# Etienne-bdt/Simple-VAE-RS

Hardware: NVIDIA B200
Metric: train patches/sec (64x64 SR CondVAE, device-timed) (higher is better)
Workload: dtype bf16

## Files before the change

### simple-vae-rs_b200/svrs_native/csrc/conv_simt.cu

```cuda
#include "common.cuh"
#include <stdlib.h>
#include "taps.cuh"
#include "tc_ptx.cuh"

namespace svrs {

struct ConvArgs {
    const void* in;
    void* out;
    const void* w;
    const float* bias;
    int act;
    double* bn_sums;
    TapGeom g;
};

constexpr int BK = 16;

}
#include "conv_narrow.cuh"
namespace svrs {
extern int g_tc_enabled_narrow;

template <typename T, int BM, int BN>
// ... 235 lines not shown
        if (dtype == SVRS_F32 && out_dtype == SVRS_F32) launch_pixel<float, float>(a, grid, st);
        else if (dtype == SVRS_BF16 && out_dtype == SVRS_BF16) launch_pixel<__nv_bfloat16, __nv_bfloat16>(a, grid, st);
        else if (dtype == SVRS_BF16 && out_dtype == SVRS_F32) launch_pixel<__nv_bfloat16, float>(a, grid, st);
        else { set_error("conv: unsupported (dtype, out_dtype) = (%d, %d)", dtype, out_dtype); return SVRS_E_UNSUPPORTED; }
        return check_launch("conv_pixel_kernel");
    }
    if (out_dtype != dtype || a.bn_sums) {
        set_error("conv: fp32 output / fused BatchNorm statistics are not available on the generic SIMT kernel (K=%d Nc=%d)", g.K, g.Nc);
        return SVRS_E_UNSUPPORTED;
    }
    if (g.Nc <= 16) {
        dim3 grid((unsigned)((M + 255) / 256), (g.Nc + 15) / 16, g.nprob);
        if (dtype == SVRS_F32) SVRS_LAUNCH((conv_taps_kernel<float, 256, 16>), grid, 256, 0, st, a);
        else SVRS_LAUNCH((conv_taps_kernel<__nv_bfloat16, 256, 16>), grid, 256, 0, st, a);
    } else {
        dim3 grid((unsigned)((M + 63) / 64), (g.Nc + 63) / 64, g.nprob);
        if (dtype == SVRS_F32) SVRS_LAUNCH((conv_taps_kernel<float, 64, 64>), grid, 256, 0, st, a);
        else SVRS_LAUNCH((conv_taps_kernel<__nv_bfloat16, 64, 64>), grid, 256, 0, st, a);
    }
    return check_launch("conv_taps_kernel");
}

struct WgradArgs {
    const void* gmat;
    const void* x;
    float* dw;
    int KK;
    int ksplit;
    TapGeom g;
};

}
#include "wgrad_narrow.cuh"
#include "wgrad16.cuh"
namespace svrs {

template <typename T>
__global__ void __launch_bounds__(256) wgrad_taps_kernel(const __grid_constant__ WgradArgs a) {
    pdl_entry();
    constexpr int BA = 64, BB = 64, BP = 16;
    __shared__ float Gs[BP][BA];
    __shared__ float Xs[BP][BB];
    const TapGeom& g = a.g;
    const Prob& pb = g.prob[0];
    const T* __restrict__ G = reinterpret_cast<const T*>(a.gmat) + pb.out_off;
    const T* __restrict__ X = reinterpret_cast<const T*>(a.x);
    const int Ca = g.Nc, Cb = g.K;
    const int b_tiles = (Cb + BB - 1) / BB;
    const int a0 = (blockIdx.x / b_tiles) * BA;
    const int b0 = (blockIdx.x % b_tiles) * BB;
    const int t = blockIdx.y;
    const Tap tp = pb.taps[t];
    const long long M = (long long)g.N * g.OH * g.OW;
    long long chunk = (M + a.ksplit - 1) / a.ksplit;
    chunk = (chunk + BP - 1) / BP * BP;
    const long long mbeg = (long long)blockIdx.z * chunk;
    const long long mend = mbeg + chunk < M ? mbeg + chunk : M;
    const int tid = threadIdx.x;
    const int tx = tid % 16, ty = tid / 16;
    const bool vecG = (Ca % 4 == 0), vecX = (Cb % 4 == 0);
    const int lp = tid / 16;
    const int lq = (tid % 16) * 4;

    float acc[4][4];
#pragma unroll
    for (int i = 0; i < 4; ++i)
#pragma unroll
// ... 511 lines not shown
    ConvArgs a;
    a.in = x; a.out = y; a.w = w_kn; a.bias = bias; a.act = act; a.bn_sums = bn_sums;
    geom_convT4s2(a.g, N, H, W, Cin, Cout);
    return launch_conv(a, dtype, (cudaStream_t)stream);
}

extern "C" int svrs_convT2d_fprop(const void* x, const void* w_kn, const void* w_nk, const float* bias, void* y, int dtype,
                                  int N, int H, int W, int Cin, int Cout, int act, void* stream) {
    return svrs_convT2d_fprop_ex(x, w_kn, w_nk, bias, y, dtype, nullptr, N, H, W, Cin, Cout, act, stream);
}

extern "C" int svrs_convT2d_dgrad(const void* dy, const void* w_kn, const void* w_nk, void* dx, int dtype,
                                  int N, int H, int W, int Cin, int Cout, void* stream) {
    SVRS_CHECK_ARG(dy && w_kn && dx && dtype_ok(dtype), "convT2d_dgrad: null pointer or bad dtype");
    if (N > 0 && use_tc(w_nk, dtype, Cout, Cin, W, H))
        return launch_conv_tc(2, dy, w_nk, nullptr, dx, N, 2 * H, 2 * W, Cout, Cin, SVRS_ACT_NONE, ConvExtra(), (cudaStream_t)stream);
    ConvArgs a;
    a.in = dy; a.out = dx; a.w = w_kn; a.bias = nullptr; a.act = SVRS_ACT_NONE; a.bn_sums = nullptr;
    geom_conv4s2(a.g, N, 2 * H, 2 * W, Cout, Cin);
    return launch_conv(a, dtype, (cudaStream_t)stream);
}

extern "C" int svrs_conv2d_wgrad(const void* x, const void* dy, float* dw, float* dw_packed, float* db, int dtype,
                                 int N, int H, int W, int Cin, int Cout, int ksize, int ksplit, void* stream) {
    SVRS_CHECK_ARG(x && dy && dtype_ok(dtype), "conv2d_wgrad: null pointer or bad dtype");
    SVRS_CHECK_ARG(ksize == 3 || (ksize == 4 && H % 2 == 0 && W % 2 == 0), "conv2d_wgrad: bad ksize");
    int rc = 0;
    if (dw) {
        WgradArgs a;
        a.gmat = dy; a.x = x; a.dw = dw; a.KK = ksize * ksize;
        if (ksize == 3) geom_conv3(a.g, N, H, W, Cin, Cout, false);
        else geom_conv4s2(a.g, N, H, W, Cin, Cout);
        const bool fold_db = db != nullptr && Cout % 8 == 0;
        if (g_tc_enabled_narrow && ksplit <= 0 && wgrad16_takes(dtype, N, H, W, Cin, Cout, ksize)) {
            rc = launch_wgrad16(x, dy, dw, db, N, H, W, Cin, (cudaStream_t)stream);
            db = nullptr;
        } else if (g_tc_enabled && N > 0 && dtype == SVRS_BF16 && wgrad_halo_supported(a.g, a.KK)) {
            rc = launch_wgrad3_halo(a.g, dy, x, dw_packed ? dw_packed : dw, dw_packed != nullptr, fold_db ? db : nullptr, (cudaStream_t)stream);
            if (fold_db) db = nullptr;
        } else if (g_tc_enabled && N > 0 && wgrad_tc_supported(dtype, Cout, Cin, a.g.OW, a.g.OH)) {
            rc = launch_wgrad_tc(a.g, dy, x, dw_packed ? dw_packed : dw, dw_packed != nullptr, a.KK, fold_db ? db : nullptr, (cudaStream_t)stream);
            if (fold_db) db = nullptr;
        } else if (g_tc_enabled_narrow && N > 0 && ksplit <= 0 && wgrad_narrow_mma_takes(a.g, dtype)) {
            rc = launch_wgrad_narrow_mma(a, db, (cudaStream_t)stream);
            db = nullptr;
        } else
            rc = launch_wgrad(a, dtype, ksplit, (cudaStream_t)stream);
        if (rc) return rc;
    }
    if (db) {
        int s = ksize == 3 ? 1 : 2;
        rc = launch_colsum(dy, dtype, (long long)N * (H / s) * (W / s), Cout, db, (cudaStream_t)stream);
    }
    return rc;
}

extern "C" int svrs_convT2d_wgrad(const void* x, const void* dy, float* dw, float* dw_packed, float* db, int dtype,
                                  int N, int H, int W, int Cin, int Cout, int ksplit, void* stream) {
    SVRS_CHECK_ARG(x && dy && dtype_ok(dtype), "convT2d_wgrad: null pointer or bad dtype");
    int rc = 0;
    if (dw) {
        WgradArgs a;
        a.gmat = x; a.x = dy; a.dw = dw; a.KK = 16;
        geom_conv4s2(a.g, N, 2 * H, 2 * W, Cout, Cin);
        if (g_tc_enabled && N > 0 && wgrad_tc_supported(dtype, Cin, Cout, a.g.OW, a.g.OH))
            rc = launch_wgrad_tc(a.g, x, dy, dw_packed ? dw_packed : dw, dw_packed != nullptr, 16, nullptr, (cudaStream_t)stream);
        else
            rc = launch_wgrad(a, dtype, ksplit, (cudaStream_t)stream);
        if (rc) return rc;
    }
    if (db) rc = launch_colsum(dy, dtype, (long long)N * 4 * H * W, Cout, db, (cudaStream_t)stream);
    return rc;
}

extern "C" int svrs_conv2d_wgrad_layout(int dtype, int N, int H, int W, int Cin, int Cout, int ksize) {
    if (!(ksize == 3 || (ksize == 4 && H % 2 == 0 && W % 2 == 0)) || N <= 0) return 0;
    if (g_tc_enabled_narrow && wgrad16_takes(dtype, N, H, W, Cin, Cout, ksize)) return 0;
    TapGeom g;
    if (ksize == 3) geom_conv3(g, N, H, W, Cin, Cout, false);
    else geom_conv4s2(g, N, H, W, Cin, Cout);
    if (g_tc_enabled && dtype == SVRS_BF16 && wgrad_halo_supported(g, ksize * ksize)) return 1;
    if (g_tc_enabled && wgrad_tc_supported(dtype, Cout, Cin, g.OW, g.OH)) return 1;
    return 0;
}
extern "C" int svrs_convT2d_wgrad_layout(int dtype, int N, int H, int W, int Cin, int Cout) {
    if (N <= 0) return 0;
    TapGeom g;
    geom_conv4s2(g, N, 2 * H, 2 * W, Cout, Cin);
    return (g_tc_enabled && wgrad_tc_supported(dtype, Cin, Cout, g.OW, g.OH)) ? 1 : 0;
}

extern "C" int svrs_debug_tap_geometry(int form, int N, int H, int W, int Cr, int Cw, int64_t* out, int cap) {
    SVRS_CHECK_ARG(out && form >= 0 && form <= 3, "debug_tap_geometry: bad args");
    TapGeom g;
    if (form == 0) geom_conv3(g, N, H, W, Cr, Cw, false);
    else if (form == 1) geom_conv3(g, N, H, W, Cr, Cw, true);
    else if (form == 2) geom_conv4s2(g, N, H, W, Cr, Cw);
    else geom_convT4s2(g, N, H, W, Cr, Cw);
    int n = 0;
    auto put = [&](long long v) { if (n < cap) out[n] = v; ++n; };
    put(g.N); put(g.OH); put(g.OW); put(g.IH); put(g.IW); put(g.K); put(g.Nc); put(g.nprob);
    put(g.o_sn); put(g.o_sy); put(g.o_sx); put(g.i_sn); put(g.i_sy); put(g.i_sx);
    for (int p = 0; p < g.nprob; ++p) {
        put(g.prob[p].out_off); put(g.prob[p].ntaps);
        for (int t = 0; t < g.prob[p].ntaps; ++t) {
            put(g.prob[p].taps[t].in_off); put(g.prob[p].taps[t].w_off); put(g.prob[p].taps[t].dy); put(g.prob[p].taps[t].dx);
        }
    }
    SVRS_CHECK_ARG(n <= cap, "debug_tap_geometry: buffer too small (%d needed)", n);
    return n;
// ... 2 lines not shown
```

### simple-vae-rs_b200/svrs_native/csrc/conv_tc.cu

```cuda
#include "common.cuh"
#include <stdlib.h>
#include "taps.cuh"
#include <cuda.h>
#include <string.h>
#include "tc_ptx.cuh"

namespace svrs {

constexpr int TC_STAGES = 4;
constexpr int TC_A_BYTES = 128 * 128;
constexpr int TC_B_BYTES = 256 * 128;
constexpr int TC_STAGE_BYTES = TC_A_BYTES + TC_B_BYTES;
constexpr int TC_SMEM_BYTES = TC_STAGES * TC_STAGE_BYTES + 1024  + 256 ;
constexpr int TC_THREADS = 64 + 32 * TC_EPI_WARPS;

struct TcTap {
    int map;
    int dy, dx;
    int wtap;
};
struct TcProb {
    int ntaps;
    int pad_;
    long long out_off;
// ... 162 lines not shown
        if (EXTRA && p.bn_sums) epi_bn_flush(s_bn, p.bn_sums, p.Nc, threadIdx.x - 64, 32 * TC_EPI_WARPS);
    }

    tc_fence_before();
    __syncthreads();
    if (warp == 1) {
        tc_fence_after();
        asm volatile("tcgen05.dealloc.cta_group::1.sync.aligned.b32 %0, 512;" ::"r"(tmem_base) : "memory");
    }
}

typedef CUresult (*PFN_encodeTiled)(CUtensorMap*, CUtensorMapDataType, cuuint32_t, void*, const cuuint64_t*, const cuuint64_t*,
                                    const cuuint32_t*, const cuuint32_t*, CUtensorMapInterleave, CUtensorMapSwizzle,
                                    CUtensorMapL2promotion, CUtensorMapFloatOOBfill);

static PFN_encodeTiled get_encode() {
    static PFN_encodeTiled fn = nullptr;
    if (!fn) {
        void* ptr = nullptr;
        cudaDriverEntryPointQueryResult qres;
        if (cudaGetDriverEntryPoint("cuTensorMapEncodeTiled", &ptr, cudaEnableDefault, &qres) == cudaSuccess && qres == cudaDriverEntryPointSuccess)
            fn = (PFN_encodeTiled)ptr;
    }
    return fn;
}

static CUtensorMapSwizzle swizzle_for(int cw) {
    return cw == 64 ? CU_TENSOR_MAP_SWIZZLE_128B : (cw == 32 ? CU_TENSOR_MAP_SWIZZLE_64B : CU_TENSOR_MAP_SWIZZLE_32B);
}

int chunk_width(int C) { return C % 64 == 0 ? 64 : (C % 32 == 0 ? 32 : (C % 16 == 0 ? 16 : 0)); }

int make_act_map(CUtensorMap* m, const void* base, int C, int W, int H, int N, long long sx, long long sy, long long sn,
                 int BW, int BH, int BNI, int cw) {
    PFN_encodeTiled enc = get_encode();
    if (!enc) { set_error("cuTensorMapEncodeTiled unavailable"); return SVRS_E_CUDA; }
    cuuint64_t dims[4] = {(cuuint64_t)C, (cuuint64_t)W, (cuuint64_t)H, (cuuint64_t)N};
    cuuint64_t strides[3] = {(cuuint64_t)sx * 2, (cuuint64_t)sy * 2, (cuuint64_t)sn * 2};
    cuuint32_t box[4] = {(cuuint32_t)cw, (cuuint32_t)BW, (cuuint32_t)BH, (cuuint32_t)BNI};
    cuuint32_t es[4] = {1, 1, 1, 1};
    CUresult r = enc(m, CU_TENSOR_MAP_DATA_TYPE_BFLOAT16, 4, const_cast<void*>(base), dims, strides, box, es,
                     CU_TENSOR_MAP_INTERLEAVE_NONE, swizzle_for(cw), CU_TENSOR_MAP_L2_PROMOTION_L2_128B,
                     CU_TENSOR_MAP_FLOAT_OOB_FILL_NONE);
    if (r != CUDA_SUCCESS) { set_error("cuTensorMapEncodeTiled(activation) failed: %d (C=%d W=%d H=%d N=%d cw=%d)", (int)r, C, W, H, N, cw); return SVRS_E_CUDA; }
    return 0;
}

int make_f32_2d_map(CUtensorMap* m, const void* base, long long inner, long long rows, int box_inner, int box_rows) {
    PFN_encodeTiled enc = get_encode();
    if (!enc) { set_error("cuTensorMapEncodeTiled unavailable"); return SVRS_E_CUDA; }
    cuuint64_t dims[2] = {(cuuint64_t)inner, (cuuint64_t)rows};
    cuuint64_t strides[1] = {(cuuint64_t)inner * 4};
    cuuint32_t box[2] = {(cuuint32_t)box_inner, (cuuint32_t)box_rows};
    cuuint32_t es[2] = {1, 1};
    CUtensorMapSwizzle sw = box_inner * 4 == 128 ? CU_TENSOR_MAP_SWIZZLE_128B : CU_TENSOR_MAP_SWIZZLE_64B;
    CUresult r = enc(m, CU_TENSOR_MAP_DATA_TYPE_FLOAT32, 2, const_cast<void*>(base), dims, strides, box, es,
                     CU_TENSOR_MAP_INTERLEAVE_NONE, sw, CU_TENSOR_MAP_L2_PROMOTION_NONE, CU_TENSOR_MAP_FLOAT_OOB_FILL_NONE);
    if (r != CUDA_SUCCESS) { set_error("cuTensorMapEncodeTiled(f32 2d) failed: %d (inner=%lld rows=%lld box %dx%d)", (int)r, inner, rows, box_inner, box_rows); return SVRS_E_CUDA; }
    return 0;
}

static int make_w_map(CUtensorMap* m, const void* base, int K, int Nc, int taps, int n_tile, int cw) {
    PFN_encodeTiled enc = get_encode();
    if (!enc) { set_error("cuTensorMapEncodeTiled unavailable"); return SVRS_E_CUDA; }
    cuuint64_t dims[3] = {(cuuint64_t)K, (cuuint64_t)Nc, (cuuint64_t)taps};
    cuuint64_t strides[2] = {(cuuint64_t)K * 2, (cuuint64_t)K * Nc * 2};
    cuuint32_t box[3] = {(cuuint32_t)cw, (cuuint32_t)n_tile, 1};
    cuuint32_t es[3] = {1, 1, 1};
    CUresult r = enc(m, CU_TENSOR_MAP_DATA_TYPE_BFLOAT16, 3, const_cast<void*>(base), dims, strides, box, es,
                     CU_TENSOR_MAP_INTERLEAVE_NONE, swizzle_for(cw), CU_TENSOR_MAP_L2_PROMOTION_L2_256B,
                     CU_TENSOR_MAP_FLOAT_OOB_FILL_NONE);
    if (r != CUDA_SUCCESS) { set_error("cuTensorMapEncodeTiled(weights) failed: %d (K=%d Nc=%d taps=%d)", (int)r, K, Nc, taps); return SVRS_E_CUDA; }
    return 0;
}

int make_plane_map_3d(CUtensorMap* m, const void* base, int elem_bytes, int S, long long planes, int box_w, int box_h, int box_c) {
// ... 118 lines not shown
```

### simple-vae-rs_b200/svrs_native/csrc/tc_ptx.cuh

```cuda
#pragma once
#include <cuda.h>
#include <stdint.h>

namespace svrs {

__device__ __forceinline__ uint32_t smem_u32(const void* p) { return (uint32_t)__cvta_generic_to_shared(p); }

__device__ __forceinline__ void mbar_init(uint32_t bar, uint32_t count) {
    asm volatile("mbarrier.init.shared::cta.b64 [%0], %1;" ::"r"(bar), "r"(count) : "memory");
}
__device__ __forceinline__ void mbar_expect_tx(uint32_t bar, uint32_t bytes) {
    asm volatile("mbarrier.arrive.expect_tx.shared::cta.b64 _, [%0], %1;" ::"r"(bar), "r"(bytes) : "memory");
}
__device__ __forceinline__ void mbar_arrive(uint32_t bar) {
    asm volatile("mbarrier.arrive.shared::cta.b64 _, [%0];" ::"r"(bar) : "memory");
}
__device__ __forceinline__ void mbar_wait(uint32_t bar, uint32_t parity) {
    asm volatile(
        "{\n\t"
        ".reg .pred P1;\n\t"
        "WAIT_LOOP:\n\t"
        "mbarrier.try_wait.parity.shared::cta.b64 P1, [%0], %1;\n\t"
        "@P1 bra DONE;\n\t"
        "bra WAIT_LOOP;\n\t"
// ... 270 lines not shown
        if (act == SVRS_ACT_HARDTANH7) epi_rows<SVRS_ACT_HARDTANH7, true, true>(taddr, n_tile, half, orow, bias, c_base, Nc, row_ok, er);
        else if (bias) epi_rows<SVRS_ACT_NONE, true, true>(taddr, n_tile, half, orow, bias, c_base, Nc, row_ok, er);
        else epi_rows<SVRS_ACT_NONE, false, true>(taddr, n_tile, half, orow, bias, c_base, Nc, row_ok, er);
        return;
    }
    if (bias) {
        if (act == SVRS_ACT_SIGMOID) epi_rows<SVRS_ACT_SIGMOID, true, false>(taddr, n_tile, half, orow, bias, c_base, Nc, row_ok, er);
        else if (act == SVRS_ACT_HARDTANH7) epi_rows<SVRS_ACT_HARDTANH7, true, false>(taddr, n_tile, half, orow, bias, c_base, Nc, row_ok, er);
        else epi_rows<SVRS_ACT_NONE, true, false>(taddr, n_tile, half, orow, bias, c_base, Nc, row_ok, er);
    } else {
        epi_rows<SVRS_ACT_NONE, false, false>(taddr, n_tile, half, orow, bias, c_base, Nc, row_ok, er);
    }
}

__device__ __forceinline__ void epi_bn_zero(float* sbn) {
    for (int i = threadIdx.x; i < 2 * EPI_BN_MAXC; i += blockDim.x) sbn[i] = 0.f;
}
__device__ __forceinline__ void epi_bn_flush(const float* sbn, double* sums, int C, int epi_tid, int epi_threads) {
    named_bar_sync(3, epi_threads);
    double* dst = sums + (size_t)(blockIdx.x % SVRS_BN_REPLICAS) * 2 * C;
    for (int c = epi_tid; c < C; c += epi_threads) {
        const float s1 = sbn[c], s2 = sbn[EPI_BN_MAXC + c];
        if (s1 != 0.f || s2 != 0.f) { atomicAdd(dst + c, (double)s1); atomicAdd(dst + C + c, (double)s2); }
    }
}

struct ConvExtra {
    float* out2 = nullptr;
    long long out2_ld = 0;
    double* bn_sums = nullptr;
};

int make_act_map(CUtensorMap* m, const void* base, int C, int W, int H, int N, long long sx, long long sy, long long sn,
                 int BW, int BH, int BNI, int cw);
bool pick_box(int OW, int OH, int& BW, int& BH, int& BNI);
int make_f32_2d_map(CUtensorMap* m, const void* base, long long inner, long long rows, int box_inner, int box_rows);
int chunk_width(int C);

}
```

### simple-vae-rs_b200/svrs_native/csrc/wgrad16.cuh

```cuda
#pragma once
#include <cooperative_groups.h>

namespace svrs {

__device__ __forceinline__ void ldsm_x4_trans(uint32_t (&r)[4], uint32_t saddr) {
    asm volatile("ldmatrix.sync.aligned.m8n8.x4.trans.shared.b16 {%0,%1,%2,%3}, [%4];"
                 : "=r"(r[0]), "=r"(r[1]), "=r"(r[2]), "=r"(r[3]) : "r"(saddr));
}

struct Wg16Args {
    const __nv_bfloat16* x;
    const __nv_bfloat16* g;
    float* dw;
    float* db;
    int N, H, W, R;
    int units, units_per_cta;
};

constexpr int WG16_THREADS = 128;

template <int CB>
__global__ void __launch_bounds__(WG16_THREADS) wgrad16_mma_kernel(const __grid_constant__ Wg16Args a) {
    pdl_entry();
    constexpr int XP = CB * 2 + 16;
    constexpr int GP = 16 * 2 + 16;
    constexpr int CHUNKS = CB / 16;
    extern __shared__ __align__(16) uint8_t smem[];
    const int W = a.W, R = a.R;
    const int xrow_bytes = (W + 2) * XP;
    uint8_t* xs = smem;
    uint8_t* gs = smem + (size_t)(R + 2) * xrow_bytes;
    const int lane = threadIdx.x & 31, warp = threadIdx.x >> 5;
    const int gq = lane >> 2, q = lane & 3;
    for (int i = threadIdx.x; i < (R + 2) * 2 * (XP / 16); i += WG16_THREADS) {
        const int row = i / (2 * (XP / 16)), rem = i % (2 * (XP / 16));
        const int side = rem / (XP / 16), c16 = rem % (XP / 16);
        *reinterpret_cast<uint4*>(xs + (size_t)row * xrow_bytes + (size_t)(side ? W + 1 : 0) * XP + c16 * 16) = make_uint4(0u, 0u, 0u, 0u);
    }
    float acc[9][2][4], accb[2][4];
#pragma unroll
    for (int t = 0; t < 9; ++t)
#pragma unroll
        for (int j = 0; j < 2; ++j)
#pragma unroll
            for (int e = 0; e < 4; ++e) acc[t][j][e] = 0.f;
#pragma unroll
    for (int j = 0; j < 2; ++j)
#pragma unroll
        for (int e = 0; e < 4; ++e) accb[j][e] = 0.f;
    const uint32_t xs_u = smem_u32(xs), gs_u = smem_u32(gs);
    const int blocks_per_img = a.H / R;
    const int mt_per_row = W / 16, mtiles = R * mt_per_row;
    const int u0 = blockIdx.x * a.units_per_cta;
    const int u1 = u0 + a.units_per_cta < a.units ? u0 + a.units_per_cta : a.units;
    const int l_pix = ((lane >> 4) & 1) * 8 + (lane & 7), l_ch8 = (lane >> 3) & 1;
    const int g_pix = ((lane >> 3) & 1) * 8 + (lane & 7), g_ch8 = (lane >> 4) & 1;
    const uint32_t ONES = 0x3F803F80u;
    for (int u = u0; u < u1; ++u) {
        const int n = u / blocks_per_img, y0 = (u % blocks_per_img) * R;
        __syncthreads();
        {
            constexpr int CPP = CB / 8;
            constexpr int PPP = WG16_THREADS / CPP;
            const int c16 = threadIdx.x % CPP, pxl = threadIdx.x / CPP;
            for (int row = 0; row < R + 2; ++row) {
                const int yy = y0 - 1 + row;
                const bool ok = yy >= 0 && yy < a.H;
                const __nv_bfloat16* src = a.x + (((long long)n * a.H + (ok ? yy : 0)) * W) * CB + c16 * 8;
                uint8_t* dst = xs + (size_t)row * xrow_bytes + XP + c16 * 16;
#pragma unroll 4
                for (int px = pxl; px < W; px += PPP) {
                    uint4 v = make_uint4(0u, 0u, 0u, 0u);
                    if (ok) v = __ldg(reinterpret_cast<const uint4*>(src + (long long)px * CB));
                    *reinterpret_cast<uint4*>(dst + (size_t)px * XP) = v;
                }
            }
            const int gc = threadIdx.x & 1, gpx = threadIdx.x >> 1;
            for (int row = 0; row < R; ++row) {
                const __nv_bfloat16* src = a.g + (((long long)n * a.H + y0 + row) * W) * 16 + gc * 8;
                uint8_t* dst = gs + (size_t)row * W * GP + gc * 16;
#pragma unroll 2
                for (int px = gpx; px < W; px += WG16_THREADS / 2)
                    *reinterpret_cast<uint4*>(dst + (size_t)px * GP) = __ldg(reinterpret_cast<const uint4*>(src + (long long)px * 16));
            }
        }
        __syncthreads();
        for (int mt = (CHUNKS == 1 ? warp : 0); mt < mtiles; mt += (CHUNKS == 1 ? 4 : 1)) {
            const int rr = mt / mt_per_row, x0 = (mt - rr * mt_per_row) * 16;
            const int chunk = CHUNKS == 1 ? 0 : warp;
            uint32_t bf[4];
            ldsm_x4_trans(bf, gs_u + (uint32_t)(((rr * W) + x0 + g_pix) * GP + g_ch8 * 16));
#pragma unroll
            for (int t = 0; t < 9; ++t) {
                const int dy = t / 3 - 1, dx = t % 3 - 1;
                uint32_t af[4];
                ldsm_x4_trans(af, xs_u + (uint32_t)((rr + 1 + dy) * xrow_bytes + (x0 + dx + 1 + l_pix) * XP + chunk * 32 + l_ch8 * 16));
                mma_bf16_16816(acc[t][0], af, bf[0], bf[1]);
                mma_bf16_16816(acc[t][1], af, bf[2], bf[3]);
            }
            if (a.db && (CHUNKS == 1 || warp == 0)) {
                const uint32_t one4[4] = {ONES, ONES, ONES, ONES};
                mma_bf16_16816(accb[0], one4, bf[0], bf[1]);
                mma_bf16_16816(accb[1], one4, bf[2], bf[3]);
            }
        }
    }
    __syncthreads();
    float* s_red = reinterpret_cast<float*>(smem);
    constexpr int NRED = 9 * CB * 16 + 16;
    for (int i = threadIdx.x; i < NRED; i += WG16_THREADS) s_red[i] = 0.f;
    __syncthreads();
    {
        const int chunk = CHUNKS == 1 ? 0 : warp;
#pragma unroll
        for (int t = 0; t < 9; ++t)
#pragma unroll
            for (int j = 0; j < 2; ++j) {
                float* dst = s_red + (t * CB + chunk * 16) * 16 + j * 8 + 2 * q;
                atomicAdd(dst + gq * 16, acc[t][j][0]);
                atomicAdd(dst + gq * 16 + 1, acc[t][j][1]);
                atomicAdd(dst + (gq + 8) * 16, acc[t][j][2]);
                atomicAdd(dst + (gq + 8) * 16 + 1, acc[t][j][3]);
            }
        if (a.db && (CHUNKS == 1 || warp == 0) && gq == 0) {
#pragma unroll
            for (int j = 0; j < 2; ++j) {
                atomicAdd(s_red + 9 * CB * 16 + j * 8 + 2 * q, accb[j][0]);
                atomicAdd(s_red + 9 * CB * 16 + j * 8 + 2 * q + 1, accb[j][1]);
            }
        }
    }
    __syncthreads();
    namespace cg = cooperative_groups;
    cg::cluster_group cluster = cg::this_cluster();
    const unsigned cs = cluster.num_blocks(), cr = cluster.block_rank();
    if (cs > 1) cluster.sync();
    for (unsigned e = cr + cs * threadIdx.x; e < (unsigned)NRED; e += cs * WG16_THREADS) {
        float v = 0.f;
        for (unsigned r = 0; r < cs; ++r) v += cs > 1 ? cluster.map_shared_rank(s_red, r)[e] : s_red[e];
        if (v == 0.f) continue;
        if (e < 9u * CB * 16u) {
            const int t = e / (CB * 16), b = (e / 16) % CB, ca = e % 16;
            atomicAdd(&a.dw[((long long)ca * CB + b) * 9 + t], v);
        } else if (a.db) {
            atomicAdd(&a.db[e - 9u * CB * 16u], v);
        }
    }
    if (cs > 1) cluster.sync();
}

static bool wgrad16_takes(int dtype, int N, int H, int W, int Cin, int Cout, int ksize) {
    if (dtype != SVRS_BF16 || ksize != 3 || Cout != 16 || !(Cin == 16 || Cin == 64) || N <= 0) return false;
    if (W % 16 != 0 || W > 64 || W < 16) return false;
    const int R = W >= 32 ? 2 : 4;
    return H % R == 0 && (long long)N * H * W < (1ll << 31);
}

static int launch_wgrad16(const void* x, const void* g, float* dw, float* db, int N, int H, int W, int Cin, cudaStream_t st) {
    Wg16Args a;
    a.x = reinterpret_cast<const __nv_bfloat16*>(x); a.g = reinterpret_cast<const __nv_bfloat16*>(g);
    a.dw = dw; a.db = db; a.N = N; a.H = H; a.W = W; a.R = W >= 32 ? 2 : 4;
    a.units = N * (H / a.R);
    static const int per_sm = getenv("SVRS_WG16_CTAS_PER_SM") ? atoi(getenv("SVRS_WG16_CTAS_PER_SM")) : 2;
    long long ctas = (long long)per_sm * num_sms();
    if (ctas > a.units) ctas = a.units;
    a.units_per_cta = (int)((a.units + ctas - 1) / ctas);
    ctas = (a.units + a.units_per_cta - 1) / a.units_per_cta;
    const int cs = ctas >= 8 ? 8 : 1;
    ctas = (ctas + cs - 1) / cs * cs;
    const int XP = Cin * 2 + 16, GP = 48;
    size_t stage = (size_t)(a.R + 2) * (W + 2) * XP + (size_t)a.R * W * GP;
    size_t red = (size_t)(9 * Cin * 16 + 16) * sizeof(float);
    size_t smem = stage > red ? stage : red;
    static bool attr_set = false;
    if (!attr_set) {
        cudaFuncSetAttribute(wgrad16_mma_kernel<16>, cudaFuncAttributeMaxDynamicSharedMemorySize, 64 * 1024);
        cudaFuncSetAttribute(wgrad16_mma_kernel<64>, cudaFuncAttributeMaxDynamicSharedMemorySize, 64 * 1024);
        attr_set = true;
    }
    if (smem > 64 * 1024) { set_error("wgrad16: staging does not fit (%zu bytes)", smem); return SVRS_E_UNSUPPORTED; }
    cudaLaunchConfig_t cfg = {};
    cfg.gridDim = dim3((unsigned)ctas);
    cfg.blockDim = dim3(WG16_THREADS);
    cfg.dynamicSmemBytes = smem;
    cfg.stream = st;
    cudaLaunchAttribute attr[1];
    attr[0].id = cudaLaunchAttributeClusterDimension;
    attr[0].val.clusterDim.x = cs; attr[0].val.clusterDim.y = 1; attr[0].val.clusterDim.z = 1;
    cfg.attrs = attr;
    cfg.numAttrs = 1;
    if (Cin == 16) cudaLaunchKernelEx(&cfg, wgrad16_mma_kernel<16>, a);
    else cudaLaunchKernelEx(&cfg, wgrad16_mma_kernel<64>, a);
    return check_launch("wgrad16_mma_kernel");
}

}
```

Measured before the change: 46740.

## Replace wgrad16 with warp-specialized TMA-pipelined tail wgrad kernel covering Cout=4

```diff
diff --git a/simple-vae-rs_b200/svrs_native/csrc/conv_simt.cu b/simple-vae-rs_b200/svrs_native/csrc/conv_simt.cu
--- a/simple-vae-rs_b200/svrs_native/csrc/conv_simt.cu
+++ b/simple-vae-rs_b200/svrs_native/csrc/conv_simt.cu
@@ -291,7 +291,7 @@
 
 }
 #include "wgrad_narrow.cuh"
-#include "wgrad16.cuh"
+#include "wgrad_tail.cuh"
 namespace svrs {
 
 template <typename T>
@@ -869,8 +869,8 @@
         if (ksize == 3) geom_conv3(a.g, N, H, W, Cin, Cout, false);
         else geom_conv4s2(a.g, N, H, W, Cin, Cout);
         const bool fold_db = db != nullptr && Cout % 8 == 0;
-        if (g_tc_enabled_narrow && ksplit <= 0 && wgrad16_takes(dtype, N, H, W, Cin, Cout, ksize)) {
-            rc = launch_wgrad16(x, dy, dw, db, N, H, W, Cin, (cudaStream_t)stream);
+        if (g_tc_enabled_narrow && ksplit <= 0 && wgrad_tail_takes(dtype, N, H, W, Cin, Cout, ksize)) {
+            rc = launch_wgrad_tail(x, dy, dw, db, N, H, W, Cin, Cout, (cudaStream_t)stream);
             db = nullptr;
         } else if (g_tc_enabled && N > 0 && dtype == SVRS_BF16 && wgrad_halo_supported(a.g, a.KK)) {
             rc = launch_wgrad3_halo(a.g, dy, x, dw_packed ? dw_packed : dw, dw_packed != nullptr, fold_db ? db : nullptr, (cudaStream_t)stream);
@@ -912,7 +912,7 @@
 
 extern "C" int svrs_conv2d_wgrad_layout(int dtype, int N, int H, int W, int Cin, int Cout, int ksize) {
     if (!(ksize == 3 || (ksize == 4 && H % 2 == 0 && W % 2 == 0)) || N <= 0) return 0;
-    if (g_tc_enabled_narrow && wgrad16_takes(dtype, N, H, W, Cin, Cout, ksize)) return 0;
+    if (g_tc_enabled_narrow && wgrad_tail_takes(dtype, N, H, W, Cin, Cout, ksize)) return 0;
     TapGeom g;
     if (ksize == 3) geom_conv3(g, N, H, W, Cin, Cout, false);
     else geom_conv4s2(g, N, H, W, Cin, Cout);
diff --git a/simple-vae-rs_b200/svrs_native/csrc/conv_tc.cu b/simple-vae-rs_b200/svrs_native/csrc/conv_tc.cu
--- a/simple-vae-rs_b200/svrs_native/csrc/conv_tc.cu
+++ b/simple-vae-rs_b200/svrs_native/csrc/conv_tc.cu
@@ -218,7 +218,7 @@
 int chunk_width(int C) { return C % 64 == 0 ? 64 : (C % 32 == 0 ? 32 : (C % 16 == 0 ? 16 : 0)); }
 
 int make_act_map(CUtensorMap* m, const void* base, int C, int W, int H, int N, long long sx, long long sy, long long sn,
-                 int BW, int BH, int BNI, int cw) {
+                 int BW, int BH, int BNI, int cw, bool swizzle) {
     PFN_encodeTiled enc = get_encode();
     if (!enc) { set_error("cuTensorMapEncodeTiled unavailable"); return SVRS_E_CUDA; }
     cuuint64_t dims[4] = {(cuuint64_t)C, (cuuint64_t)W, (cuuint64_t)H, (cuuint64_t)N};
@@ -226,8 +226,8 @@
     cuuint32_t box[4] = {(cuuint32_t)cw, (cuuint32_t)BW, (cuuint32_t)BH, (cuuint32_t)BNI};
     cuuint32_t es[4] = {1, 1, 1, 1};
     CUresult r = enc(m, CU_TENSOR_MAP_DATA_TYPE_BFLOAT16, 4, const_cast<void*>(base), dims, strides, box, es,
-                     CU_TENSOR_MAP_INTERLEAVE_NONE, swizzle_for(cw), CU_TENSOR_MAP_L2_PROMOTION_L2_128B,
-                     CU_TENSOR_MAP_FLOAT_OOB_FILL_NONE);
+                     CU_TENSOR_MAP_INTERLEAVE_NONE, swizzle ? swizzle_for(cw) : CU_TENSOR_MAP_SWIZZLE_NONE,
+                     CU_TENSOR_MAP_L2_PROMOTION_L2_128B, CU_TENSOR_MAP_FLOAT_OOB_FILL_NONE);
     if (r != CUDA_SUCCESS) { set_error("cuTensorMapEncodeTiled(activation) failed: %d (C=%d W=%d H=%d N=%d cw=%d)", (int)r, C, W, H, N, cw); return SVRS_E_CUDA; }
     return 0;
 }
diff --git a/simple-vae-rs_b200/svrs_native/csrc/tc_ptx.cuh b/simple-vae-rs_b200/svrs_native/csrc/tc_ptx.cuh
--- a/simple-vae-rs_b200/svrs_native/csrc/tc_ptx.cuh
+++ b/simple-vae-rs_b200/svrs_native/csrc/tc_ptx.cuh
@@ -326,7 +326,7 @@
 };
 
 int make_act_map(CUtensorMap* m, const void* base, int C, int W, int H, int N, long long sx, long long sy, long long sn,
-                 int BW, int BH, int BNI, int cw);
+                 int BW, int BH, int BNI, int cw, bool swizzle = true);
 bool pick_box(int OW, int OH, int& BW, int& BH, int& BNI);
 int make_f32_2d_map(CUtensorMap* m, const void* base, long long inner, long long rows, int box_inner, int box_rows);
 int chunk_width(int C);
diff --git a/simple-vae-rs_b200/svrs_native/csrc/wgrad16.cuh b/simple-vae-rs_b200/svrs_native/csrc/wgrad16.cuh
--- a/simple-vae-rs_b200/svrs_native/csrc/wgrad16.cuh
+++ /dev/null
@@ -1,197 +0,0 @@
-#pragma once
-#include <cooperative_groups.h>
-
-namespace svrs {
-
-__device__ __forceinline__ void ldsm_x4_trans(uint32_t (&r)[4], uint32_t saddr) {
-    asm volatile("ldmatrix.sync.aligned.m8n8.x4.trans.shared.b16 {%0,%1,%2,%3}, [%4];"
-                 : "=r"(r[0]), "=r"(r[1]), "=r"(r[2]), "=r"(r[3]) : "r"(saddr));
-}
-
-struct Wg16Args {
-    const __nv_bfloat16* x;
-    const __nv_bfloat16* g;
-    float* dw;
-    float* db;
-    int N, H, W, R;
-    int units, units_per_cta;
-};
-
-constexpr int WG16_THREADS = 128;
-
-template <int CB>
-__global__ void __launch_bounds__(WG16_THREADS) wgrad16_mma_kernel(const __grid_constant__ Wg16Args a) {
-    pdl_entry();
-    constexpr int XP = CB * 2 + 16;
-    constexpr int GP = 16 * 2 + 16;
-    constexpr int CHUNKS = CB / 16;
-    extern __shared__ __align__(16) uint8_t smem[];
-    const int W = a.W, R = a.R;
-    const int xrow_bytes = (W + 2) * XP;
-    uint8_t* xs = smem;
-    uint8_t* gs = smem + (size_t)(R + 2) * xrow_bytes;
-    const int lane = threadIdx.x & 31, warp = threadIdx.x >> 5;
-    const int gq = lane >> 2, q = lane & 3;
-    for (int i = threadIdx.x; i < (R + 2) * 2 * (XP / 16); i += WG16_THREADS) {
-        const int row = i / (2 * (XP / 16)), rem = i % (2 * (XP / 16));
-        const int side = rem / (XP / 16), c16 = rem % (XP / 16);
-        *reinterpret_cast<uint4*>(xs + (size_t)row * xrow_bytes + (size_t)(side ? W + 1 : 0) * XP + c16 * 16) = make_uint4(0u, 0u, 0u, 0u);
-    }
-    float acc[9][2][4], accb[2][4];
-#pragma unroll
-    for (int t = 0; t < 9; ++t)
-#pragma unroll
-        for (int j = 0; j < 2; ++j)
-#pragma unroll
-            for (int e = 0; e < 4; ++e) acc[t][j][e] = 0.f;
-#pragma unroll
-    for (int j = 0; j < 2; ++j)
-#pragma unroll
-        for (int e = 0; e < 4; ++e) accb[j][e] = 0.f;
-    const uint32_t xs_u = smem_u32(xs), gs_u = smem_u32(gs);
-    const int blocks_per_img = a.H / R;
-    const int mt_per_row = W / 16, mtiles = R * mt_per_row;
-    const int u0 = blockIdx.x * a.units_per_cta;
-    const int u1 = u0 + a.units_per_cta < a.units ? u0 + a.units_per_cta : a.units;
-    const int l_pix = ((lane >> 4) & 1) * 8 + (lane & 7), l_ch8 = (lane >> 3) & 1;
-    const int g_pix = ((lane >> 3) & 1) * 8 + (lane & 7), g_ch8 = (lane >> 4) & 1;
-    const uint32_t ONES = 0x3F803F80u;
-    for (int u = u0; u < u1; ++u) {
-        const int n = u / blocks_per_img, y0 = (u % blocks_per_img) * R;
-        __syncthreads();
-        {
-            constexpr int CPP = CB / 8;
-            constexpr int PPP = WG16_THREADS / CPP;
-            const int c16 = threadIdx.x % CPP, pxl = threadIdx.x / CPP;
-            for (int row = 0; row < R + 2; ++row) {
-                const int yy = y0 - 1 + row;
-                const bool ok = yy >= 0 && yy < a.H;
-                const __nv_bfloat16* src = a.x + (((long long)n * a.H + (ok ? yy : 0)) * W) * CB + c16 * 8;
-                uint8_t* dst = xs + (size_t)row * xrow_bytes + XP + c16 * 16;
-#pragma unroll 4
-                for (int px = pxl; px < W; px += PPP) {
-                    uint4 v = make_uint4(0u, 0u, 0u, 0u);
-                    if (ok) v = __ldg(reinterpret_cast<const uint4*>(src + (long long)px * CB));
-                    *reinterpret_cast<uint4*>(dst + (size_t)px * XP) = v;
-                }
-            }
-            const int gc = threadIdx.x & 1, gpx = threadIdx.x >> 1;
-            for (int row = 0; row < R; ++row) {
-                const __nv_bfloat16* src = a.g + (((long long)n * a.H + y0 + row) * W) * 16 + gc * 8;
-                uint8_t* dst = gs + (size_t)row * W * GP + gc * 16;
-#pragma unroll 2
-                for (int px = gpx; px < W; px += WG16_THREADS / 2)
-                    *reinterpret_cast<uint4*>(dst + (size_t)px * GP) = __ldg(reinterpret_cast<const uint4*>(src + (long long)px * 16));
-            }
-        }
-        __syncthreads();
-        for (int mt = (CHUNKS == 1 ? warp : 0); mt < mtiles; mt += (CHUNKS == 1 ? 4 : 1)) {
-            const int rr = mt / mt_per_row, x0 = (mt - rr * mt_per_row) * 16;
-            const int chunk = CHUNKS == 1 ? 0 : warp;
-            uint32_t bf[4];
-            ldsm_x4_trans(bf, gs_u + (uint32_t)(((rr * W) + x0 + g_pix) * GP + g_ch8 * 16));
-#pragma unroll
-            for (int t = 0; t < 9; ++t) {
-                const int dy = t / 3 - 1, dx = t % 3 - 1;
-                uint32_t af[4];
-                ldsm_x4_trans(af, xs_u + (uint32_t)((rr + 1 + dy) * xrow_bytes + (x0 + dx + 1 + l_pix) * XP + chunk * 32 + l_ch8 * 16));
-                mma_bf16_16816(acc[t][0], af, bf[0], bf[1]);
-                mma_bf16_16816(acc[t][1], af, bf[2], bf[3]);
-            }
-            if (a.db && (CHUNKS == 1 || warp == 0)) {
-                const uint32_t one4[4] = {ONES, ONES, ONES, ONES};
-                mma_bf16_16816(accb[0], one4, bf[0], bf[1]);
-                mma_bf16_16816(accb[1], one4, bf[2], bf[3]);
-            }
-        }
-    }
-    __syncthreads();
-    float* s_red = reinterpret_cast<float*>(smem);
-    constexpr int NRED = 9 * CB * 16 + 16;
-    for (int i = threadIdx.x; i < NRED; i += WG16_THREADS) s_red[i] = 0.f;
-    __syncthreads();
-    {
-        const int chunk = CHUNKS == 1 ? 0 : warp;
-#pragma unroll
-        for (int t = 0; t < 9; ++t)
-#pragma unroll
-            for (int j = 0; j < 2; ++j) {
-                float* dst = s_red + (t * CB + chunk * 16) * 16 + j * 8 + 2 * q;
-                atomicAdd(dst + gq * 16, acc[t][j][0]);
-                atomicAdd(dst + gq * 16 + 1, acc[t][j][1]);
-                atomicAdd(dst + (gq + 8) * 16, acc[t][j][2]);
-                atomicAdd(dst + (gq + 8) * 16 + 1, acc[t][j][3]);
-            }
-        if (a.db && (CHUNKS == 1 || warp == 0) && gq == 0) {
-#pragma unroll
-            for (int j = 0; j < 2; ++j) {
-                atomicAdd(s_red + 9 * CB * 16 + j * 8 + 2 * q, accb[j][0]);
-                atomicAdd(s_red + 9 * CB * 16 + j * 8 + 2 * q + 1, accb[j][1]);
-            }
-        }
-    }
-    __syncthreads();
-    namespace cg = cooperative_groups;
-    cg::cluster_group cluster = cg::this_cluster();
-    const unsigned cs = cluster.num_blocks(), cr = cluster.block_rank();
-    if (cs > 1) cluster.sync();
-    for (unsigned e = cr + cs * threadIdx.x; e < (unsigned)NRED; e += cs * WG16_THREADS) {
-        float v = 0.f;
-        for (unsigned r = 0; r < cs; ++r) v += cs > 1 ? cluster.map_shared_rank(s_red, r)[e] : s_red[e];
-        if (v == 0.f) continue;
-        if (e < 9u * CB * 16u) {
-            const int t = e / (CB * 16), b = (e / 16) % CB, ca = e % 16;
-            atomicAdd(&a.dw[((long long)ca * CB + b) * 9 + t], v);
-        } else if (a.db) {
-            atomicAdd(&a.db[e - 9u * CB * 16u], v);
-        }
-    }
-    if (cs > 1) cluster.sync();
-}
-
-static bool wgrad16_takes(int dtype, int N, int H, int W, int Cin, int Cout, int ksize) {
-    if (dtype != SVRS_BF16 || ksize != 3 || Cout != 16 || !(Cin == 16 || Cin == 64) || N <= 0) return false;
-    if (W % 16 != 0 || W > 64 || W < 16) return false;
-    const int R = W >= 32 ? 2 : 4;
-    return H % R == 0 && (long long)N * H * W < (1ll << 31);
-}
-
-static int launch_wgrad16(const void* x, const void* g, float* dw, float* db, int N, int H, int W, int Cin, cudaStream_t st) {
-    Wg16Args a;
-    a.x = reinterpret_cast<const __nv_bfloat16*>(x); a.g = reinterpret_cast<const __nv_bfloat16*>(g);
-    a.dw = dw; a.db = db; a.N = N; a.H = H; a.W = W; a.R = W >= 32 ? 2 : 4;
-    a.units = N * (H / a.R);
-    static const int per_sm = getenv("SVRS_WG16_CTAS_PER_SM") ? atoi(getenv("SVRS_WG16_CTAS_PER_SM")) : 2;
-    long long ctas = (long long)per_sm * num_sms();
-    if (ctas > a.units) ctas = a.units;
-    a.units_per_cta = (int)((a.units + ctas - 1) / ctas);
-    ctas = (a.units + a.units_per_cta - 1) / a.units_per_cta;
-    const int cs = ctas >= 8 ? 8 : 1;
-    ctas = (ctas + cs - 1) / cs * cs;
-    const int XP = Cin * 2 + 16, GP = 48;
-    size_t stage = (size_t)(a.R + 2) * (W + 2) * XP + (size_t)a.R * W * GP;
-    size_t red = (size_t)(9 * Cin * 16 + 16) * sizeof(float);
-    size_t smem = stage > red ? stage : red;
-    static bool attr_set = false;
-    if (!attr_set) {
-        cudaFuncSetAttribute(wgrad16_mma_kernel<16>, cudaFuncAttributeMaxDynamicSharedMemorySize, 64 * 1024);
-        cudaFuncSetAttribute(wgrad16_mma_kernel<64>, cudaFuncAttributeMaxDynamicSharedMemorySize, 64 * 1024);
-        attr_set = true;
-    }
-    if (smem > 64 * 1024) { set_error("wgrad16: staging does not fit (%zu bytes)", smem); return SVRS_E_UNSUPPORTED; }
-    cudaLaunchConfig_t cfg = {};
-    cfg.gridDim = dim3((unsigned)ctas);
-    cfg.blockDim = dim3(WG16_THREADS);
-    cfg.dynamicSmemBytes = smem;
-    cfg.stream = st;
-    cudaLaunchAttribute attr[1];
-    attr[0].id = cudaLaunchAttributeClusterDimension;
-    attr[0].val.clusterDim.x = cs; attr[0].val.clusterDim.y = 1; attr[0].val.clusterDim.z = 1;
-    cfg.attrs = attr;
-    cfg.numAttrs = 1;
-    if (Cin == 16) cudaLaunchKernelEx(&cfg, wgrad16_mma_kernel<16>, a);
-    else cudaLaunchKernelEx(&cfg, wgrad16_mma_kernel<64>, a);
-    return check_launch("wgrad16_mma_kernel");
-}
-
-}
diff --git a/simple-vae-rs_b200/svrs_native/csrc/wgrad_tail.cuh b/simple-vae-rs_b200/svrs_native/csrc/wgrad_tail.cuh
--- /dev/null
+++ b/simple-vae-rs_b200/svrs_native/csrc/wgrad_tail.cuh
@@ -0,0 +1,262 @@
+#pragma once
+#include <cooperative_groups.h>
+
+namespace svrs {
+
+__device__ __forceinline__ void ldsm_x4_trans(uint32_t (&r)[4], uint32_t saddr) {
+    asm volatile("ldmatrix.sync.aligned.m8n8.x4.trans.shared.b16 {%0,%1,%2,%3}, [%4];"
+                 : "=r"(r[0]), "=r"(r[1]), "=r"(r[2]), "=r"(r[3]) : "r"(saddr));
+}
+__device__ __forceinline__ uint32_t lds_u32(uint32_t saddr) {
+    uint32_t v;
+    asm volatile("ld.shared.u32 %0, [%1];" : "=r"(v) : "r"(saddr));
+    return v;
+}
+__device__ __forceinline__ void bulk_load_g2s(uint32_t dst, const void* src, uint32_t bytes, uint32_t bar) {
+    asm volatile("cp.async.bulk.shared::cluster.global.mbarrier::complete_tx::bytes [%0], [%1], %2, [%3];"
+                 ::"r"(dst), "l"(src), "r"(bytes), "r"(bar) : "memory");
+}
+
+constexpr int WT_CONSUMERS = 8;
+constexpr int WT_THREADS = 32 * (WT_CONSUMERS + 1);
+constexpr int WT_MAX_STAGES = 8;
+
+struct WgTailArgs {
+    CUtensorMap x_map;
+    const __nv_bfloat16* g;
+    float* dw;
+    float* db;
+    int H, W, R;
+    int units, units_per_cta;
+    int stages;
+    uint32_t stage_bytes;
+};
+
+template <int CB, int CG>
+__global__ void __launch_bounds__(WT_THREADS, 1) wgrad_tail_kernel(const __grid_constant__ WgTailArgs a) {
+    pdl_entry();
+    constexpr int XP = CB * 2 + 16;
+    constexpr int GP = CG * 2;
+    constexpr int NT = CG == 16 ? 2 : 1;
+    constexpr int CHUNKS = CB / 16;
+    constexpr int PG = WT_CONSUMERS / CHUNKS;
+    extern __shared__ uint8_t smem_raw[];
+    __shared__ __align__(8) uint64_t full_bar[WT_MAX_STAGES], empty_bar[WT_MAX_STAGES];
+    const uint32_t raw_u = smem_u32(smem_raw), base_u = (raw_u + 127u) & ~127u;
+    uint8_t* smem = smem_raw + (base_u - raw_u);
+    const int W = a.W, R = a.R, S = a.stages;
+    const uint32_t xbox = (uint32_t)((R + 2) * (W + 2) * XP);
+    const int blocks_per_img = (a.H + R - 1) / R;
+    const int u0 = blockIdx.x * a.units_per_cta;
+    const int u1 = u0 + a.units_per_cta < a.units ? u0 + a.units_per_cta : a.units;
+    const int lane = threadIdx.x & 31, warp = threadIdx.x >> 5;
+    if (threadIdx.x == 0) {
+        for (int s = 0; s < S; ++s) {
+            mbar_init(smem_u32(&full_bar[s]), 1);
+            mbar_init(smem_u32(&empty_bar[s]), WT_CONSUMERS);
+        }
+        asm volatile("fence.mbarrier_init.release.cluster;" ::: "memory");
+    }
+    __syncthreads();
+
+    float acc[9][NT][4], accb[NT][4];
+#pragma unroll
+    for (int t = 0; t < 9; ++t)
+#pragma unroll
+        for (int j = 0; j < NT; ++j)
+#pragma unroll
+            for (int e = 0; e < 4; ++e) acc[t][j][e] = 0.f;
+#pragma unroll
+    for (int j = 0; j < NT; ++j)
+#pragma unroll
+        for (int e = 0; e < 4; ++e) accb[j][e] = 0.f;
+    const int gq = lane >> 2, q = lane & 3;
+    const int chunk = warp % CHUNKS;
+
+    if (warp == WT_CONSUMERS) {
+        if (lane == 0 && u0 < u1) {
+            prefetch_tmap(&a.x_map);
+            for (int u = u0, i = 0; u < u1; ++u, ++i) {
+                const int s = i % S;
+                if (i >= S) mbar_wait(smem_u32(&empty_bar[s]), ((i / S) & 1) ^ 1);
+                const int n = u / blocks_per_img, y0 = (u % blocks_per_img) * R;
+                const int rv = a.H - y0 < R ? a.H - y0 : R;
+                const uint32_t gbytes = (uint32_t)(rv * W * GP);
+                const uint32_t dst = base_u + (uint32_t)s * a.stage_bytes, bar = smem_u32(&full_bar[s]);
+                mbar_expect_tx(bar, xbox + gbytes);
+                tma_load_4d(dst, &a.x_map, bar, 0, -1, y0 - 1, n);
+                bulk_load_g2s(dst + xbox, a.g + ((long long)n * a.H + y0) * W * CG, gbytes, bar);
+            }
+        }
+        __syncwarp();
+    } else {
+        const int pg = warp / CHUNKS;
+        const int xrow_bytes = (W + 2) * XP;
+        const int mt_per_row = W / 16;
+        const int l_pix = ((lane >> 4) & 1) * 8 + (lane & 7), l_ch8 = (lane >> 3) & 1;
+        const int g_pix = ((lane >> 3) & 1) * 8 + (lane & 7), g_ch8 = (lane >> 4) & 1;
+        const uint32_t g4_off = (uint32_t)(2 * q * GP + (gq & 2) * 2), g4_sel = (gq & 1) ? 0x7632u : 0x5410u;
+        const uint32_t ONES = 0x3F803F80u;
+        const uint32_t lane_x = (uint32_t)((l_pix + 1) * XP + chunk * 32 + l_ch8 * 16);
+        for (int u = u0, i = 0; u < u1; ++u, ++i) {
+            const int s = i % S;
+            const int y0 = (u % blocks_per_img) * R;
+            const int rv = a.H - y0 < R ? a.H - y0 : R;
+            const uint32_t xs_u = base_u + (uint32_t)s * a.stage_bytes, gs_u = xs_u + xbox;
+            mbar_wait(smem_u32(&full_bar[s]), (i / S) & 1);
+            const int mtiles = rv * mt_per_row;
+            for (int mt = pg; mt < mtiles; mt += PG) {
+                const int rr = mt / mt_per_row, x0 = (mt - rr * mt_per_row) * 16;
+                uint32_t bf[2 * NT];
+                if (CG == 16) {
+                    uint32_t t4[4];
+                    ldsm_x4_trans(t4, gs_u + (uint32_t)((rr * W + x0 + g_pix) * GP + g_ch8 * 16));
+#pragma unroll
+                    for (int e = 0; e < 2 * NT; ++e) bf[e] = t4[e];
+                } else {
+                    const uint32_t ga = gs_u + (uint32_t)((rr * W + x0) * GP) + g4_off;
+                    const uint32_t lo = __byte_perm(lds_u32(ga), lds_u32(ga + GP), g4_sel);
+                    const uint32_t hi = __byte_perm(lds_u32(ga + 8 * GP), lds_u32(ga + 9 * GP), g4_sel);
+                    bf[0] = gq < 4 ? lo : 0u;
+                    bf[1] = gq < 4 ? hi : 0u;
+                }
+                const uint32_t xa = xs_u + (uint32_t)((rr + 1) * xrow_bytes + x0 * XP) + lane_x;
+#pragma unroll
+                for (int t = 0; t < 9; ++t) {
+                    const int dy = t / 3 - 1, dx = t % 3 - 1;
+                    uint32_t af[4];
+                    ldsm_x4_trans(af, xa + (uint32_t)(dy * xrow_bytes + dx * XP));
+#pragma unroll
+                    for (int j = 0; j < NT; ++j) mma_bf16_16816(acc[t][j], af, bf[2 * j], bf[2 * j + 1]);
+                }
+                if (a.db && chunk == 0) {
+                    const uint32_t one4[4] = {ONES, ONES, ONES, ONES};
+#pragma unroll
+                    for (int j = 0; j < NT; ++j) mma_bf16_16816(accb[j], one4, bf[2 * j], bf[2 * j + 1]);
+                }
+            }
+            __syncwarp();
+            if (lane == 0) mbar_arrive(smem_u32(&empty_bar[s]));
+        }
+    }
+    __syncthreads();
+    float* s_red = reinterpret_cast<float*>(smem);
+    constexpr int NRED = 9 * CB * CG + CG;
+    for (int i = threadIdx.x; i < NRED; i += WT_THREADS) s_red[i] = 0.f;
+    __syncthreads();
+    if (warp < WT_CONSUMERS) {
+#pragma unroll
+        for (int t = 0; t < 9; ++t)
+#pragma unroll
+            for (int j = 0; j < NT; ++j) {
+                if (j * 8 + 2 * q >= CG) continue;
+                float* dst = s_red + (t * CB + chunk * 16) * CG + j * 8 + 2 * q;
+                atomicAdd(dst + gq * CG, acc[t][j][0]);
+                atomicAdd(dst + gq * CG + 1, acc[t][j][1]);
+                atomicAdd(dst + (gq + 8) * CG, acc[t][j][2]);
+                atomicAdd(dst + (gq + 8) * CG + 1, acc[t][j][3]);
+            }
+        if (a.db && chunk == 0 && gq == 0) {
+#pragma unroll
+            for (int j = 0; j < NT; ++j) {
+                if (j * 8 + 2 * q >= CG) continue;
+                atomicAdd(s_red + 9 * CB * CG + j * 8 + 2 * q, accb[j][0]);
+                atomicAdd(s_red + 9 * CB * CG + j * 8 + 2 * q + 1, accb[j][1]);
+            }
+        }
+    }
+    __syncthreads();
+    namespace cg = cooperative_groups;
+    cg::cluster_group cluster = cg::this_cluster();
+    const unsigned cs = cluster.num_blocks(), cr = cluster.block_rank();
+    if (cs > 1) cluster.sync();
+    for (unsigned e = cr + cs * threadIdx.x; e < (unsigned)NRED; e += cs * WT_THREADS) {
+        float v = 0.f;
+        for (unsigned r = 0; r < cs; ++r) v += cs > 1 ? cluster.map_shared_rank(s_red, r)[e] : s_red[e];
+        if (v == 0.f) continue;
+        if (e < 9u * CB * CG) {
+            const int t = e / (CB * CG), b = (e / CG) % CB, ca = e % CG;
+            atomicAdd(&a.dw[((long long)ca * CB + b) * 9 + t], v);
+        } else if (a.db) {
+            atomicAdd(&a.db[e - 9u * CB * CG], v);
+        }
+    }
+    if (cs > 1) cluster.sync();
+}
+
+static bool wgrad_tail_takes(int dtype, int N, int H, int W, int Cin, int Cout, int ksize) {
+    if (dtype != SVRS_BF16 || ksize != 3 || N <= 0 || H <= 0) return false;
+    if (!((Cout == 16 && (Cin == 16 || Cin == 64)) || (Cout == 4 && Cin == 16))) return false;
+    return W % 16 == 0 && W >= 16 && W <= 64 && (long long)N * H * W < (1ll << 31);
+}
+
+constexpr size_t WT_SMEM_BUDGET = 220 * 1024;
+
+template <int CB, int CG>
+static int launch_wgrad_tail_t(const void* x, const void* g, float* dw, float* db, int N, int H, int W, cudaStream_t st) {
+    if (((uintptr_t)x | (uintptr_t)g) % 16) { set_error("wgrad_tail: x and dy must be 16-byte aligned"); return SVRS_E_UNSUPPORTED; }
+    WgTailArgs a;
+    a.g = reinterpret_cast<const __nv_bfloat16*>(g);
+    a.dw = dw; a.db = db; a.H = H; a.W = W;
+    a.R = 256 / W < H ? 256 / W : H;
+    const int blocks_per_img = (H + a.R - 1) / a.R;
+    a.units = N * blocks_per_img;
+    const size_t xbox = (size_t)(a.R + 2) * (W + 2) * (CB * 2 + 16);
+    a.stage_bytes = (uint32_t)((xbox + (size_t)a.R * W * CG * 2 + 127) / 128 * 128);
+    a.stages = (int)(WT_SMEM_BUDGET / a.stage_bytes);
+    if (a.stages > WT_MAX_STAGES) a.stages = WT_MAX_STAGES;
+    if (a.stages < 2) { set_error("wgrad_tail: staging does not fit (%u bytes per stage)", a.stage_bytes); return SVRS_E_UNSUPPORTED; }
+    size_t smem = (size_t)a.stages * a.stage_bytes;
+    const size_t red = (size_t)(9 * CB * CG + CG) * sizeof(float);
+    if (red > smem) smem = red;
+    smem += 128;
+    int rc = make_act_map(&a.x_map, x, CB, W, H, N, CB, (long long)W * CB, (long long)H * W * CB, W + 2, a.R + 2, 1, CB + 8, false);
+    if (rc) return rc;
+    cudaLaunchConfig_t cfg = {};
+    cfg.blockDim = dim3(WT_THREADS);
+    cfg.dynamicSmemBytes = smem;
+    cfg.stream = st;
+    cudaLaunchAttribute attr[1];
+    attr[0].id = cudaLaunchAttributeClusterDimension;
+    attr[0].val.clusterDim.y = 1; attr[0].val.clusterDim.z = 1;
+    cfg.attrs = attr;
+    cfg.numAttrs = 1;
+    constexpr int MAX_DEV = 64;
+    static int cached_cs_dev[MAX_DEV] = {}, cached_ctas_dev[MAX_DEV] = {};
+    int dev = 0;
+    if (cudaGetDevice(&dev) != cudaSuccess || dev < 0 || dev >= MAX_DEV) { set_error("wgrad_tail: no usable current device"); return SVRS_E_CUDA; }
+    int& cached_cs = cached_cs_dev[dev];
+    int& cached_ctas = cached_ctas_dev[dev];
+    if (!cached_cs) {
+        cudaFuncSetAttribute(wgrad_tail_kernel<CB, CG>, cudaFuncAttributeMaxDynamicSharedMemorySize, (int)(WT_SMEM_BUDGET + 128));
+        cached_cs = 1;
+        cudaDeviceGetAttribute(&cached_ctas, cudaDevAttrMultiProcessorCount, dev);
+        cudaLaunchConfig_t q = cfg;
+        q.dynamicSmemBytes = WT_SMEM_BUDGET + 128;
+        for (int cs : {8, 4, 2}) {
+            q.gridDim = dim3((unsigned)(cs * 64));
+            attr[0].val.clusterDim.x = cs;
+            int nc = 0;
+            if (cudaOccupancyMaxActiveClusters(&nc, wgrad_tail_kernel<CB, CG>, &q) != cudaSuccess) { cudaGetLastError(); nc = 0; }
+            if (nc * cs > (cached_cs == 1 ? 0 : cached_ctas)) { cached_cs = cs; cached_ctas = nc * cs; }
+        }
+    }
+    long long ctas = cached_ctas;
+    if (ctas > a.units) ctas = a.units;
+    a.units_per_cta = (int)((a.units + ctas - 1) / ctas);
+    ctas = (a.units + a.units_per_cta - 1) / a.units_per_cta;
+    const int cs = ctas >= cached_cs ? cached_cs : 1;
+    ctas = (ctas + cs - 1) / cs * cs;
+    cfg.gridDim = dim3((unsigned)ctas);
+    attr[0].val.clusterDim.x = cs;
+    cudaLaunchKernelEx(&cfg, wgrad_tail_kernel<CB, CG>, a);
+    return check_launch("wgrad_tail_kernel");
+}
+
+static int launch_wgrad_tail(const void* x, const void* g, float* dw, float* db, int N, int H, int W, int Cin, int Cout, cudaStream_t st) {
+    if (Cout == 4) return launch_wgrad_tail_t<16, 4>(x, g, dw, db, N, H, W, st);
+    if (Cin == 16) return launch_wgrad_tail_t<16, 16>(x, g, dw, db, N, H, W, st);
+    return launch_wgrad_tail_t<64, 16>(x, g, dw, db, N, H, W, st);
+}
+
+}
```

Measured after the change: 49160 (median of 6 runs). +5.2%, better.
